# zhaowenlan1779/hekaton-system

Measured on AMD Instinct MI355X. Metric: subcircuit Groth16 proofs/sec (whole node), big-merkle, higher is better.
Workload: dtype u32 limbs (Montgomery mod-p integers)

## Files before the change

hekaton_system_amd/csrc/ntt.cuh:

```cuda
#pragma once
#include "field.cuh"

namespace hk {

constexpr int NTT_TILE_LOG = 11;
constexpr int NTT_THREADS = 512;
constexpr int POW_TABLE_BITS = 11;
constexpr int POW_TABLE_SIZE = 1 << POW_TABLE_BITS;

#if defined(__HIPCC__)

template <class Fr>
__device__ __forceinline__ Fr fr_load(const Fr* p) {
    Fr r;
    const uint4* s = reinterpret_cast<const uint4*>(p);
    uint4 a = s[0], b = s[1];
    r.v[0] = a.x; r.v[1] = a.y; r.v[2] = a.z; r.v[3] = a.w;
    r.v[4] = b.x; r.v[5] = b.y; r.v[6] = b.z; r.v[7] = b.w;
    return r;
}
template <class Fr>
__device__ __forceinline__ void fr_store(Fr* p, const Fr& lazy) {
    Fr r = Fr::canon(lazy);
    uint4* d = reinterpret_cast<uint4*>(p);
// ... 9 lines not shown
    for (u32 k = 0; k < nbits; k++)
        if ((i >> k) & 1) acc = Fr::mul(acc, fr_load(&sq[k]));
    fr_store(&tw[i], acc);
}

template <class Fr>
__device__ __forceinline__ Fr pow_from_tables(const Fr* __restrict__ pw, u32 j, u32 logn) {
    Fr g = fr_load(&pw[j & (POW_TABLE_SIZE - 1)]);
    if (logn > POW_TABLE_BITS) g = Fr::mul(g, fr_load(&pw[POW_TABLE_SIZE + ((j >> POW_TABLE_BITS) & (POW_TABLE_SIZE - 1))]));
    if (logn > 2 * POW_TABLE_BITS) g = Fr::mul(g, fr_load(&pw[2 * POW_TABLE_SIZE + (j >> (2 * POW_TABLE_BITS))]));
    return g;
}

template <class Fr>
__global__ void k_stage_tables(Fr* __restrict__ tws, const Fr* __restrict__ tw, u32 log_table) {
    size_t i = (size_t)blockIdx.x * blockDim.x + threadIdx.x;
    if ((i + 1) >> log_table) return;
    u32 s = 31 - __clz((u32)(i + 1));
    size_t j = i + 1 - ((size_t)1 << s);
    fr_store(&tws[i], fr_load(&tw[j << (log_table - s - 1)]));
}

template <class Fr, int DIT>
__global__ void __launch_bounds__(NTT_THREADS)
k_ntt_pass4(Fr* __restrict__ data, size_t stride_vec, const Fr* __restrict__ tws, u32 logn, u32 lo, u32 nst,
            u32 cols_bits, int post, u32 npost, Fr scale, const Fr* __restrict__ pw, const Fr* __restrict__ sub,
            Fr kc) {
    extern __shared__ uint4 lds_raw[];
    Fr* lds = reinterpret_cast<Fr*>(lds_raw);
    const u32 nthr = blockDim.x;
    if (blockIdx.y >= npost) post = 0;
    Fr* vec = data + (size_t)blockIdx.y * stride_vec;
    const u32 cols = 1u << cols_bits;
    const u32 tile_elems = 1u << (nst + cols_bits);
    const u32 mid_bits = lo - cols_bits;
    const u32 mid = blockIdx.x & ((1u << mid_bits) - 1u);
    const size_t base = ((size_t)(blockIdx.x >> mid_bits) << (lo + nst)) | ((size_t)mid << cols_bits);
    for (u32 e = threadIdx.x; e < tile_elems; e += nthr) {
        u32 r = e >> cols_bits, c = e & (cols - 1);
        lds[e] = fr_load(&vec[base | ((size_t)r << lo) | c]);
    }
    __syncthreads();
    const u32 npair = nst >> 1;
    for (u32 k = 0; k < npair; k++) {
        const u32 l = DIT ? 2 * k : nst - 2 - 2 * k;
        const u32 s = lo + l;
        const Fr* t_lo = tws + (((size_t)1 << s) - 1);
        const Fr* t_hi = tws + (((size_t)2 << s) - 1);
        for (u32 q = threadIdx.x; q < (tile_elems >> 2); q += nthr) {
            u32 c = q & (cols - 1), rr = q >> cols_bits;
            u32 r0 = ((rr >> l) << (l + 2)) | (rr & ((1u << l) - 1u));
            u32 j = (u32)((base | ((size_t)r0 << lo) | c) & (((size_t)1 << s) - 1));
            Fr wc = fr_load(&t_lo[j]);
            Fr wa = fr_load(&t_hi[j]);
            Fr wb = fr_load(&t_hi[j + (1u << s)]);
            u32 i0 = (r0 << cols_bits) | c, st = 1u << (l + cols_bits);
            Fr x0 = lds[i0], x1 = lds[i0 + st], x2 = lds[i0 + 2 * st], x3 = lds[i0 + 3 * st];
            if (DIT) {
                Fr v = Fr::mul(x1, wc), u = Fr::mul(x3, wc);
                x1 = Fr::sub(x0, v); x0 = Fr::add(x0, v);
                x3 = Fr::sub(x2, u); x2 = Fr::add(x2, u);
                v = Fr::mul(x2, wa); u = Fr::mul(x3, wb);
                x2 = Fr::sub(x0, v); x0 = Fr::add(x0, v);
                x3 = Fr::sub(x1, u); x1 = Fr::add(x1, u);
            } else {
                Fr v = Fr::sub(x0, x2), u = Fr::sub(x1, x3);
                x0 = Fr::add(x0, x2); x1 = Fr::add(x1, x3);
                x2 = Fr::mul(v, wa); x3 = Fr::mul(u, wb);
                v = Fr::sub(x0, x1); u = Fr::sub(x2, x3);
                x0 = Fr::add(x0, x1); x2 = Fr::add(x2, x3);
                x1 = Fr::mul(v, wc); x3 = Fr::mul(u, wc);
            }
            lds[i0] = x0; lds[i0 + st] = x1; lds[i0 + 2 * st] = x2; lds[i0 + 3 * st] = x3;
        }
        __syncthreads();
    }
    if (nst & 1) {
        const u32 l = DIT ? nst - 1 : 0;
        const u32 s = lo + l;
        const Fr* t_lo = tws + (((size_t)1 << s) - 1);
        for (u32 q = threadIdx.x; q < (tile_elems >> 1); q += nthr) {
            u32 c = q & (cols - 1), rr = q >> cols_bits;
            u32 r0 = ((rr >> l) << (l + 1)) | (rr & ((1u << l) - 1u));
            u32 j = (u32)((base | ((size_t)r0 << lo) | c) & (((size_t)1 << s) - 1));
            Fr w = fr_load(&t_lo[j]);
            u32 i0 = (r0 << cols_bits) | c, st = 1u << (l + cols_bits);
            Fr x0 = lds[i0], x1 = lds[i0 + st];
            if (DIT) {
                Fr v = Fr::mul(x1, w);
                lds[i0] = Fr::add(x0, v);
                lds[i0 + st] = Fr::sub(x0, v);
            } else {
                lds[i0] = Fr::add(x0, x1);
                lds[i0 + st] = Fr::mul(Fr::sub(x0, x1), w);
            }
        }
        __syncthreads();
    }
    for (u32 e = threadIdx.x; e < tile_elems; e += nthr) {
        u32 r = e >> cols_bits, c = e & (cols - 1);
        size_t gi = base | ((size_t)r << lo) | c;
        Fr x = lds[e];
        if (post & 2) x = Fr::mul(x, pow_from_tables(pw, logn ? (__brev((u32)gi) >> (32 - logn)) : 0u, logn));
        if (post & 4) x = Fr::sub(x, Fr::mul(fr_load(&sub[gi]), kc));
        if (post & 1) x = Fr::mul(x, scale);
        fr_store(&vec[gi], x);
    }
}

template <class Fr>
__global__ void k_scale_pow(Fr* __restrict__ data, size_t stride_vec, const Fr* __restrict__ pw, Fr scale,
                            u32 logn, int bitrev_index, int use_pow) {
    size_t pos = (size_t)blockIdx.x * blockDim.x + threadIdx.x;
    if (pos >> logn) return;
    Fr* vec = data + (size_t)blockIdx.y * stride_vec;
    Fr x = fr_load(&vec[pos]);
    x = Fr::mul(x, scale);
    if (use_pow) {
        u32 j = bitrev_index ? (logn ? (__brev((u32)pos) >> (32 - logn)) : 0u) : (u32)pos;
        x = Fr::mul(x, pow_from_tables(pw, j, logn));
    }
    fr_store(&vec[pos], x);
}

template <class Fr>
__global__ void k_bitrev(Fr* __restrict__ data, u32 logn) {
    size_t pos = (size_t)blockIdx.x * blockDim.x + threadIdx.x;
    if (pos >> logn) return;
    u32 r = logn ? (__brev((u32)pos) >> (32 - logn)) : 0u;
// ... 6 lines not shown

template <class Fr>
__global__ void k_spmv(const u64* __restrict__ row_ptr, const u32* __restrict__ col,
                       const Fr* __restrict__ val, const Fr* __restrict__ z, Fr* __restrict__ out,
                       u32 n_rows, u32 n_copy, u32 m) {
    u32 row = blockIdx.x * blockDim.x + threadIdx.x;
    if (row >= m) return;
    if (row >= n_rows) {
        fr_store(&out[row], row - n_rows < n_copy ? fr_load(&z[row - n_rows]) : Fr::zero());
        return;
    }
    u64 b = row_ptr[row], e = row_ptr[row + 1];
    Fr acc = Fr::zero();
    Fr one = Fr::one();
    for (u64 k = b; k < e; k++) {
        Fr c = fr_load(&val[k]);
        Fr x = fr_load(&z[col[k]]);
        if (!(c == one)) x = Fr::mul(x, c);
        acc = Fr::add(acc, x);
    }
    fr_store(&out[row], acc);
}

template <int UNUSED>
__global__ void k_csr_check(const u64* __restrict__ row_ptr, const u32* __restrict__ col, u64 n_rows, u64 nnz,
                            u32 n_cols, u32* __restrict__ bad) {
    u64 t = (u64)blockIdx.x * blockDim.x + threadIdx.x, stride = (u64)gridDim.x * blockDim.x;
    u32 f = 0;
    for (u64 i = t; i < n_rows; i += stride) {
        u64 b = row_ptr[i], e = row_ptr[i + 1];
        if (b > e || e > nnz) f = 1;
    }
    for (u64 k = t; k < nnz; k += stride)
        if (col[k] >= n_cols) f = 2;
    if (t == 0 && (row_ptr[0] != 0 || row_ptr[n_rows] != nnz)) f = 3;
    if (f) atomicOr(bad, f);
}

template <class Fr>
__global__ void k_copy_inputs(Fr* __restrict__ a, const Fr* __restrict__ z, u32 n_c, u32 n_inst) {
    u32 j = blockIdx.x * blockDim.x + threadIdx.x;
    if (j < n_inst) fr_store(&a[n_c + j], fr_load(&z[j]));
}

template <class Fr>
__global__ void k_mul_pointwise(Fr* __restrict__ a, const Fr* __restrict__ b, size_t m) {
// ... 9 lines not shown
```

hekaton_system_amd/csrc/prove_impl.cuh:

```cuda
#pragma once
#include <string>
#include "curve_ops_impl.cuh"
#include "ntt.cuh"
#include "fixed_base.cuh"
#include "witness.cuh"
#include "endo.cuh"

namespace hk {

template <class Fr>
static Fr host_halve(const Fr& a) {
    u32 t[Fr::N + 1];
    u64 c = 0;
    bool odd = a.v[0] & 1;
    for (int i = 0; i < Fr::N; i++) {
        c += (u64)a.v[i] + (odd ? Fr::Params::MOD[i] : 0u);
        t[i] = (u32)c;
        c >>= 32;
    }
    t[Fr::N] = (u32)c;
    Fr r;
    for (int i = 0; i < Fr::N; i++) r.v[i] = (t[i] >> 1) | (t[i + 1] << 31);
    return r;
}
template <class Fr>
static Fr host_from_limbs(const u32* l) {
    Fr r;
    for (int i = 0; i < Fr::N; i++) r.v[i] = l[i];
    return r;
}

struct NttTables {
    std::mutex mu;
    u32 log_table = 0;
    void* tw_fwd = nullptr;
    void* tw_inv = nullptr;
    void* pw_g = nullptr;
    void* pw_ginv = nullptr;
    std::vector<void*> retired;
};

template <class C>
struct NttHost {
    typedef typename C::Fr Fr;

    static hk_status ensure(hk_ctx* ctx, u32 log_m, NttTables** out) {
        if (log_m > C::TWO_ADICITY) return HK_ERR_DOMAIN_TOO_LARGE;
        std::unique_lock<std::mutex> lk(ctx->mu);
        if (!ctx->ntt) ctx->ntt = new NttTables();
        NttTables* T = ctx->ntt;
        lk.unlock();
        std::unique_lock<std::mutex> tl(T->mu);
        *out = T;
        if (T->log_table >= log_m && T->tw_fwd) return HK_OK;
        u32 L = log_m < 16 ? 16 : log_m;
        if (L > C::TWO_ADICITY) L = C::TWO_ADICITY;
        HK_HIP(hipSetDevice(ctx->device));
        std::vector<Fr> sq(32), sqi(32);
        Fr w = host_from_limbs<Fr>(C::ROOT);
        for (u32 k = 0; k < C::TWO_ADICITY - L; k++) w = Fr::sqr(w);
        Fr winv = Fr::one();
// ... 42 lines not shown
        return HK_OK;
    }

    static Fr size_inv(u32 log_m) {
        Fr x = Fr::one();
        for (u32 k = 0; k < log_m; k++) x = host_halve(x);
        return x;
    }
    static Fr vanishing_inv_on_coset(u32 log_m) {
        Fr g = host_from_limbs<Fr>(C::GEN);
        for (u32 k = 0; k < log_m; k++) g = Fr::sqr(g);
        return fp_inv(Fr::sub(g, Fr::one()));
    }

    struct Post {
        int post = 0;
        u32 nvec = 0xffffffffu;
        const Fr* scale = nullptr;
        const Fr* pw = nullptr;
        const Fr* sub = nullptr;
        const Fr* kc = nullptr;
    };

    static hk_status passes(hipStream_t s, Fr* data, size_t stride, u32 batch, u32 logn, const Fr* tws, int dit,
                            const Post& ep = Post()) {
        if (logn == 0) return HK_OK;
        static const u32 upper_max = [] {
            const char* e = getenv("HK_NTT_UPPER_MAX");
            u32 v = e ? (u32)atoi(e) : 6u;
            return v < 1 ? 1u : (v > 10 ? 10u : v);
        }();
        static const u32 tile_log = [] {
            const char* e = getenv("HK_NTT_TILE_LOG");
            u32 v = e ? (u32)atoi(e) : (u32)NTT_TILE_LOG;
            return v < 8 ? 8u : (v > (u32)NTT_TILE_LOG ? (u32)NTT_TILE_LOG : v);
        }();
        const u32 threads = 1u << (tile_log - 2);
        u32 bottom = logn < tile_log ? logn : tile_log;
        u32 rest = logn - bottom;
        u32 npass = (rest + upper_max - 1) / upper_max;
        struct P { u32 lo, nst, cols_bits; } ps[34];
        int np = 0;
        ps[np++] = {0, bottom, 0};
        u32 lo = bottom;
        for (u32 i = 0; i < npass; i++) {
            u32 nst = (rest - (lo - bottom) + (npass - i) - 1) / (npass - i);
            ps[np++] = {lo, nst, tile_log - nst};
            lo += nst;
        }
        Fr one = Fr::one();
        for (int k = 0; k < np; k++) {
            const P& p = dit ? ps[k] : ps[np - 1 - k];
            u32 tile_log = p.nst + p.cols_bits;
            dim3 grid(1u << (logn - tile_log), batch);
            size_t lds = sizeof(Fr) << tile_log;
            bool last = k == np - 1;
            int pp = last ? ep.post : 0;
            const Fr& sc = (pp & 1) ? *ep.scale : one;
            const Fr& kc = (pp & 4) ? *ep.kc : one;
            if (dit)
                hipLaunchKernelGGL((k_ntt_pass4<Fr, 1>), grid, dim3(threads), lds, s, data, stride, tws, logn, p.lo,
                                   p.nst, p.cols_bits, pp, ep.nvec, sc, ep.pw, ep.sub, kc);
            else
                hipLaunchKernelGGL((k_ntt_pass4<Fr, 0>), grid, dim3(threads), lds, s, data, stride, tws, logn, p.lo,
                                   p.nst, p.cols_bits, pp, ep.nvec, sc, ep.pw, ep.sub, kc);
        }
        HK_HIP(hipGetLastError());
        return HK_OK;
    }

    static hk_status scale(hipStream_t s, Fr* data, size_t stride, u32 batch, u32 logn, const Fr* pw,
                           const Fr& sc, int bitrev_index, int use_pow) {
        size_t n = (size_t)1 << logn;
        hipLaunchKernelGGL((k_scale_pow<Fr>), dim3((u32)((n + 255) / 256), batch), dim3(256), 0, s, data,
                           stride, pw, sc, logn, bitrev_index, use_pow);
        HK_HIP(hipGetLastError());
        return HK_OK;
    }
    static hk_status bitrev(hipStream_t s, Fr* data, u32 logn) {
        size_t n = (size_t)1 << logn;
        hipLaunchKernelGGL((k_bitrev<Fr>), dim3((u32)((n + 255) / 256)), dim3(256), 0, s, data, logn);
        HK_HIP(hipGetLastError());
        return HK_OK;
    }
};

template <class C>
hk_status Ops<C>::ntt(hk_ctx* ctx, void* data, unsigned log_m, int inverse, int coset) {
    typedef NttHost<C> N;
    NttTables* T;
// ... 35 lines not shown
    HK_HIP(hipMemsetAsync(flag, 0, sizeof(u32), s));
    size_t work = M.n_rows > M.nnz ? M.n_rows : M.nnz;
    u32 blocks = (u32)std::min<size_t>((work + 255) / 256, 2048);
    if (blocks == 0) blocks = 1;
    hipLaunchKernelGGL((k_csr_check<0>), dim3(blocks), dim3(256), 0, s, M.row_ptr, M.col, (u64)M.n_rows, (u64)M.nnz,
                       (u32)n_cols, flag);
    u32 h = 0;
    HK_HIP(hipMemcpyAsync(&h, flag, sizeof(u32), hipMemcpyDeviceToHost, s));
    HK_HIP(hipStreamSynchronize(s));
    return h ? HK_ERR_ARG : HK_OK;
}

template <class C>
struct QapHost {
    typedef typename C::Fr Fr;
    typedef NttHost<C> N;

    static u32 domain_log(size_t n_c, size_t n_inst) {
        size_t need = n_c + n_inst;
        u32 lg = 0;
        while (((size_t)1 << lg) < need) lg++;
        return lg;
    }
    static hk_status run(hipStream_t s, NttTables* T, const CsrDev& A, const CsrDev& B, const CsrDev& Cm,
                         size_t n_inst, size_t n_c, const Fr* z, Fr* abc, u32 log_m) {
        size_t m = (size_t)1 << log_m;
        const CsrDev* Ms[3] = {&A, &B, &Cm};
        for (int k = 0; k < 3; k++) {
            hipLaunchKernelGGL((k_spmv<Fr>), dim3((u32)((m + 255) / 256)), dim3(256), 0, s,
                               Ms[k]->row_ptr, Ms[k]->col, (const Fr*)Ms[k]->val, z, abc + k * m,
                               (u32)n_c, k == 0 ? (u32)n_inst : 0u, (u32)m);
        }
        const Fr* tinv = (const Fr*)T->tw_inv;
        const Fr* tfwd = (const Fr*)T->tw_fwd;
        typename N::Post e1;
        e1.post = 2;
        e1.nvec = 2;
        e1.pw = (const Fr*)T->pw_g;
        HK_TRY(N::passes(s, abc, m, 3, log_m, tinv, 0, e1));
        HK_TRY(N::passes(s, abc, m, 2, log_m, tfwd, 1));
        hipLaunchKernelGGL((k_mul_pointwise<Fr>), dim3((u32)((m + 255) / 256)), dim3(256), 0, s, abc, abc + m, m);
        Fr minv = N::size_inv(log_m);
        Fr mm = fp_inv(Fr::mul(minv, minv));
        Fr k = Fr::mul(N::vanishing_inv_on_coset(log_m), Fr::mul(minv, Fr::mul(minv, minv)));
        typename N::Post e2;
        e2.post = 2 | 4 | 1;
        e2.pw = (const Fr*)T->pw_ginv;
        e2.sub = abc + 2 * m;
        e2.kc = &mm;
        e2.scale = &k;
        HK_TRY(N::passes(s, abc, m, 1, log_m, tinv, 0, e2));
        HK_HIP(hipGetLastError());
        return HK_OK;
    }
};

template <class C>
hk_status Ops<C>::witness_map(hk_ctx* ctx, const hk_csr* A, const hk_csr* B, const hk_csr* Cm, size_t n_inst,
                              size_t n_c, const void* z, size_t n_v, void* h_out, size_t h_cap,
                              size_t* m_out) {
    typedef QapHost<C> Q;
    if (A->n_rows != n_c || B->n_rows != n_c || Cm->n_rows != n_c || n_inst > n_v || n_inst < 1) return HK_ERR_ARG;
    for (auto M : {A, B, Cm})
        if (!M->row_ptr || (M->nnz && (!M->col || !M->val_mont))) return HK_ERR_ARG;
    u32 log_m = Q::domain_log(n_c, n_inst);
    if (log_m > C::TWO_ADICITY) return HK_ERR_DOMAIN_TOO_LARGE;
    size_t m = (size_t)1 << log_m;
    if (m_out) *m_out = m;
    if (h_cap < m) return HK_ERR_LEN;
    NttTables* T;
    HK_TRY(NttHost<C>::ensure(ctx, log_m, &T));
    LaneGuard g(ctx);
    Lane* L = g.lane;
    if (!L) return HK_ERR_DEVICE;
    const hk_csr* Ms[3] = {A, B, Cm};
    const void *rp[3], *cl[3], *vl[3], *zd;
    u32* flag;
    Fr* abc;
    HK_TRY(L->carve([&](Carve& c) {
        for (int k = 0; k < 3; k++) {
            rp[k] = c.take(8 * (Ms[k]->n_rows + 1));
            cl[k] = c.take(4 * Ms[k]->nnz);
            vl[k] = c.take(sizeof(Fr) * Ms[k]->nnz);
        }
        flag = c.n<u32>(1);
        zd = c.take(n_v * sizeof(Fr));
        abc = c.n<Fr>(3 * m);
    }));
    CsrDev D[3];
    for (int k = 0; k < 3; k++) {
        HK_TRY(to_device(L, Ms[k]->row_ptr, 8 * (Ms[k]->n_rows + 1), &rp[k]));
        HK_TRY(to_device(L, Ms[k]->col, 4 * Ms[k]->nnz, &cl[k]));
        HK_TRY(to_device(L, Ms[k]->val_mont, sizeof(Fr) * Ms[k]->nnz, &vl[k]));
        D[k] = {(const u64*)rp[k], (const u32*)cl[k], vl[k], Ms[k]->n_rows, Ms[k]->nnz};
// ... 965 lines not shown
                HK_HIP(hipMemcpyAsync(t, src, k * sizeof(F), hipMemcpyHostToDevice, L->stream));
                sd = t;
            }
            F* dd = out_dev ? dst : u;
            hipLaunchKernelGGL(k_field_convert<F>, dim3((unsigned)((k + 255) / 256)), dim3(256), 0, L->stream, sd, dd, k, to_mont);
            HK_HIP(hipGetLastError());
            if (!out_dev) HK_HIP(hipMemcpyAsync(dst, dd, k * sizeof(F), hipMemcpyDeviceToHost, L->stream));
            HK_TRY(L->settle());
        }
        return HK_OK;
    };
    return which == 0 ? run(Fr()) : run(Fq());
}

template <class C>
void Ops<C>::ctx_release(hk_ctx* ctx) {
    for (auto& e : ctx->fb_cache)
        if (e.table) (void)hipFree(e.table);
    ctx->fb_cache.clear();
    if (!ctx->ntt) return;
    NttTables* T = ctx->ntt;
    for (void* p : {T->tw_fwd, T->tw_inv, T->pw_g, T->pw_ginv})
        if (p) (void)hipFree(p);
    for (void* p : T->retired) (void)hipFree(p);
    delete T;
    ctx->ntt = nullptr;
}

template <class Fr>
__global__ void k_prep_ext(Fr* __restrict__ ext, u32 ext_stride, const Fr* __restrict__ rs_kappas, u32 rs_stride,
                           u32 n_kappas, u32 batch, u32* __restrict__ c0, u32* __restrict__ c1, u32* __restrict__ c2,
                           u32 nb0, u32 nb1, u32 nb2) {
    u32 gt = blockIdx.x * blockDim.x + threadIdx.x, stride = gridDim.x * blockDim.x;
    for (u32 i = gt; i < nb0; i += stride) c0[i] = 0;
    for (u32 i = gt; i < nb1; i += stride) c1[i] = 0;
    for (u32 i = gt; i < nb2; i += stride) c2[i] = 0;
    if (gt >= batch) return;
    Fr* e = ext + (size_t)gt * ext_stride;
    const Fr* rk = rs_kappas + (size_t)gt * rs_stride;
    Fr r = fr_load(&rk[0]), s = fr_load(&rk[1]);
    fr_store(&e[0], r);
    fr_store(&e[1], s);
    fr_store(&e[2], Fr::mul(r, s));
    for (u32 i = 0; i < n_kappas; i++) fr_store(&e[3 + i], fr_load(&rk[2 + i]));
}

// ... 180 lines not shown
    }
    return HK_OK;
}

template <class C>
hk_status Ops<C>::prove_batch(hk_ctx* ctx, const hk_pk* h, size_t n_v, size_t n_kappas, const ProveRow* rows, size_t batch) {
    typedef QapHost<C> Q;
    if (h->ctx != ctx) return HK_ERR_ARG;
    PkImpl<C>* pk = (PkImpl<C>*)h->impl;
    if (!pk->has_qap) return HK_ERR_ARG;
    if (n_v != pk->n_v) return HK_ERR_LEN;
    if (n_kappas + 1 != pk->n_stages) return HK_ERR_LEN;
    if (batch == 0) return HK_OK;
    if (!rows) return HK_ERR_ARG;
    for (size_t b = 0; b < batch; b++) {
        const ProveRow& w = rows[b];
        if (!w.z || !w.r || !w.s || !w.a || !w.b || !w.c || (n_kappas && !w.kappas)) return HK_ERR_ARG;
    }
    LaneGuard g(ctx, ProveLaneTag{});
    Lane* L = g.lane;
    if (!L) return HK_ERR_DEVICE;
    NttTables* T;
    HK_TRY(NttHost<C>::ensure(ctx, pk->log_m, &T));
    const MsmPlan &pz = pk->plan_z, &ph = pk->plan_h, &pb = pk->plan_b;
    const size_t m = (size_t)1 << pk->log_m, fr = sizeof(Fr), rs_stride = 2 + n_kappas;
    std::vector<char> z_dev(batch);
    bool any_host = false;
    for (size_t b = 0; b < batch; b++) {
        z_dev[b] = is_device_ptr(rows[b].z);
        any_host = any_host || !z_dev[b];
    }
    Fr *zext, *small, *zt, *zb, *abc;
    SortBufs sb, sbh, sbb;
    typename MsmRun<Fq>::Bufs rbA, rbB1, rbL, rbh;
    typename MsmRun<Fq2>::Bufs rb2;
    XYZZ<Fq>* res1;
    XYZZ<Fq2>* res2;
    Affine<Fq> *oa, *oc;
    Affine<Fq2>* ob;
    XYZZ<Fq>* pc;
    auto chunk_bufs = [&](Carve& c, u32 nb) {
        zext = c.n<Fr>((size_t)pk->n_ext * nb);
        small = c.n<Fr>(rs_stride * nb);
        zt = any_host ? c.n<Fr>(n_v * nb) : nullptr;
        MsmSort<Fr>::alloc(c, pz, &sb, nb);
        MsmSort<Fr>::alloc(c, ph, &sbh, nb);
// ... 19 lines not shown
    size_t chunk = batch < (size_t)HK_PROVE_BATCH_CHUNK ? batch : (size_t)HK_PROVE_BATCH_CHUNK;
    if (chunk > 1) {
        size_t free_b = 0, total_b = 0;
        if (hipMemGetInfo(&free_b, &total_b) != hipSuccess) { (void)hipGetLastError(); free_b = 0; }
        size_t avail = free_b + L->arena_cap;
        auto chunk_bytes = [&](size_t nb) { Carve c; chunk_bufs(c, (u32)nb); return c.off; };
        while (chunk > 1 && chunk_bytes(chunk) > avail) chunk--;
    }
    std::vector<unsigned char> rsk(batch * rs_stride * fr);
    for (size_t b = 0; b < batch; b++) {
        unsigned char* row = rsk.data() + b * rs_stride * fr;
        memcpy(row, rows[b].r, fr);
        memcpy(row + fr, rows[b].s, fr);
        if (n_kappas) memcpy(row + 2 * fr, rows[b].kappas, n_kappas * fr);
    }
    std::vector<Affine<Fq>> ha(chunk), hc(chunk);
    std::vector<Affine<Fq2>> hb(chunk);
    std::vector<const Fr*> zd(chunk);
    const bool prof = ctx->profiling;
    hipEvent_t* ev = L->ev;
    hk_timings acc;
    memset(&acc, 0, sizeof(acc));
    static const EndoSplit<2> endo_g1 = EndoOf<Fq>::split();
    hipStream_t rs[PROVE_ROLES];
    for (int r = 0; r < PROVE_ROLES; r++) rs[r] = L->stream_at(prove_role_stream(L->n_streams, (ProveRole)r));
    hipStream_t s = rs[ROLE_MAIN];
    auto wait = [](hipStream_t to, hipEvent_t e, hipStream_t from) -> hk_status {
        if (to != from) HK_HIP(hipStreamWaitEvent(to, e, 0));
        return HK_OK;
    };
    for (size_t b0 = 0; b0 < batch; b0 += chunk) {
        const u32 nb = (u32)std::min(chunk, batch - b0);
        HK_TRY(L->carve([&](Carve& c) { chunk_bufs(c, nb); }));
        hipEvent_t ev_start = b0 ? ev[9] : ev[0];
        if (prof) HK_HIP(hipEventRecord(ev_start, s));
        for (u32 j = 0; j < nb; j++) {
            if (z_dev[b0 + j]) zd[j] = (const Fr*)rows[b0 + j].z;
            else {
                HK_HIP(hipMemcpyAsync(zt + (size_t)j * n_v, rows[b0 + j].z, n_v * fr, hipMemcpyHostToDevice, s));
                zd[j] = zt + (size_t)j * n_v;
            }
            if (n_v > 1)
                HK_HIP(hipMemcpyAsync(zext + (size_t)j * pk->n_ext, zd[j] + 1, (n_v - 1) * fr, hipMemcpyDeviceToDevice, s));
        }
        HK_HIP(hipMemcpyAsync(small, rsk.data() + b0 * rs_stride * fr, nb * rs_stride * fr, hipMemcpyHostToDevice, s));
        hipLaunchKernelGGL((k_prep_ext<Fr>), dim3(64), dim3(256), 0, s, zext + (n_v - 1), pk->n_ext, (const Fr*)small,
                           (u32)rs_stride, (u32)n_kappas, nb, sb.count, sbh.count, sbb.count, pz.NB * nb, ph.NB * nb,
                           pk->b_compact ? pb.NB * nb : 0u);
        hipStream_t sB1 = rs[ROLE_B1], sB2 = rs[ROLE_B2], sL = rs[ROLE_L], sH = rs[ROLE_H];
        hipEvent_t ev_z = ev[16], ev_sorted = ev[17];
        HK_HIP(hipEventRecord(ev_z, s));
        auto submit_h = [&]() -> hk_status {
            HK_TRY(wait(sH, ev_z, s));
            if (prof) HK_HIP(hipEventRecord(ev[5], sH));
            for (u32 j = 0; j < nb; j++)
                HK_TRY(Q::run(sH, T, pk->csr[0], pk->csr[1], pk->csr[2], pk->n_inst, pk->n_c, zd[j],
                              abc + (size_t)j * 3 * m, pk->log_m));
            if (prof) HK_HIP(hipEventRecord(ev[6], sH));
            HK_TRY(MsmSort<Fr>::run(sH, ph, (const u32*)abc, 1, sbh, true, nb, 3 * m));
            HK_TRY(MsmRun<Fq>::run(sH, ph, pk->h_tab, (u32)m, 0, sbh, rbh, res1 + 3, prof ? ev[12] : nullptr,
                                   prof ? ev[13] : nullptr, nb, 4));
            HK_HIP(hipEventRecord(ev[7], sH));
            return HK_OK;
        };
        const bool h_first = L->n_streams >= 3;
        if (h_first) HK_TRY(submit_h());
        HK_TRY(MsmSort<Fr>::run(s, pz, (const u32*)zext, 1, sb, true, nb, pk->n_ext));
        HK_HIP(hipEventRecord(ev_sorted, s));
        if (prof) HK_HIP(hipEventRecord(ev[1], s));
        HK_TRY(wait(sL, ev_sorted, s));
        const SortBufs* sbB = &sb;
        if (pk->b_compact) {
            HK_TRY(wait(sB1, ev_z, s));
            hipLaunchKernelGGL((k_gather<Fr>), dim3((pk->b_n + 255) / 256, nb), dim3(256), 0, sB1, zb, (const Fr*)zext,
                               (const u32*)pk->b_idx, pk->b_n, pk->n_ext);
            HK_TRY(MsmSort<Fr>::run(sB1, pb, (const u32*)zb, 1, sbb, true, nb, pk->b_n));
            HK_HIP(hipEventRecord(ev[28], sB1));
            HK_TRY(wait(sB2, ev[28], sB1));
            sbB = &sbb;
        } else {
            HK_TRY(wait(sB1, ev_sorted, s));
// ... 12 lines not shown
        if (prof) HK_HIP(hipEventRecord(ev[2], s));
        HK_TRY(wait(s, ev[3], sB1));
        HK_TRY(wait(s, ev[4], sB2));
        HK_TRY(wait(s, ev[18], sL));
        hipLaunchKernelGGL((k_finish_ab<Fr, Fq, Fq2>), dim3(3, nb), dim3(64), 0, s, res1, res2, pk->consts_g1, pk->consts_g2,
                           (const Fr*)small, (u32)rs_stride, oa, ob, pc, endo_g1);
        HK_HIP(hipGetLastError());
        if (!h_first) HK_TRY(submit_h());
        HK_TRY(wait(s, ev[7], sH));
        if (prof) HK_HIP(hipEventRecord(ev[19], s));
        hipLaunchKernelGGL((k_finish_c<Fq>), dim3(1), dim3(64), 0, s, (const XYZZ<Fq>*)pc, (const XYZZ<Fq>*)res1, oc, nb);
        HK_HIP(hipGetLastError());
        HK_HIP(hipMemcpyAsync(ha.data(), oa, nb * sizeof(Affine<Fq>), hipMemcpyDeviceToHost, s));
        HK_HIP(hipMemcpyAsync(hb.data(), ob, nb * sizeof(Affine<Fq2>), hipMemcpyDeviceToHost, s));
        HK_HIP(hipMemcpyAsync(hc.data(), oc, nb * sizeof(Affine<Fq>), hipMemcpyDeviceToHost, s));
        if (prof) HK_HIP(hipEventRecord(ev[8], s));
        HK_TRY(L->settle());
        for (u32 j = 0; j < nb; j++) {
            memcpy(rows[b0 + j].a, &ha[j], sizeof(Affine<Fq>));
            memcpy(rows[b0 + j].b, &hb[j], sizeof(Affine<Fq2>));
            memcpy(rows[b0 + j].c, &hc[j], sizeof(Affine<Fq>));
        }
        if (prof) {
            acc.digits_ms += ev_ms(ev_start, ev[1]);
            acc.msm_a_ms += ev_ms(ev[1], ev[2]);
            hipEvent_t fork_b = pk->b_compact ? ev_z : ev[1];
            acc.msm_b_g1_ms += ev_ms(fork_b, ev[3]);
            acc.msm_b_g2_ms += ev_ms(fork_b, ev[4]);
            acc.msm_l_ms += ev_ms(ev[1], ev[18]);
            acc.witness_map_ms += ev_ms(ev[5], ev[6]);
            acc.msm_h_ms += ev_ms(ev[6], ev[7]);
            acc.finish_ms += ev_ms(ev[19], ev[8]);
            float kh = ev_ms(ev[12], ev[13]);
            acc.accum_h_ms += kh;
            acc.accum_kernel_ms += kh + ev_ms(ev[22], ev[23]) + ev_ms(ev[24], ev[25]) + ev_ms(ev[26], ev[27]);
            acc.accum_kernel_launches += 4;
        }
    }
    if (prof) {
        acc.total_ms = ev_ms(ev[0], ev[8]);
        acc.batch_proofs = (uint32_t)chunk;
        L->timings = acc;
    }
    return HK_OK;
}

}
// ... 3 lines not shown
```

Baseline: 125.0.

## Fuse witness-map NTT seams, batch SpMV, and skip trivial twiddle multiplies

Restructures the witness-map (H polynomial) pipeline. Adjacent inverse and forward NTT passes at the bottom and top seams are fused into single kernels, so one kernel does inverse NTT, coset shift and forward NTT on an LDS-resident tile. The top seam also folds the pointwise A*B product and the following inverse NTT into one kernel. The three SpMVs become one launch, the closing scale is folded into a precomputed power table, and stage-0 butterflies skip multiplies by one. This removes several global-memory round trips and kernel launches, at the cost of more complex kernels and a new plan helper. It also adds an optional split of the witness maps onto the main stream.

```diff
diff --git a/hekaton_system_amd/csrc/ntt.cuh b/hekaton_system_amd/csrc/ntt.cuh
--- a/hekaton_system_amd/csrc/ntt.cuh
+++ b/hekaton_system_amd/csrc/ntt.cuh
@@ -55,31 +55,42 @@
 }
 
 template <class Fr, int DIT>
-__global__ void __launch_bounds__(NTT_THREADS)
-k_ntt_pass4(Fr* __restrict__ data, size_t stride_vec, const Fr* __restrict__ tws, u32 logn, u32 lo, u32 nst,
-            u32 cols_bits, int post, u32 npost, Fr scale, const Fr* __restrict__ pw, const Fr* __restrict__ sub,
-            Fr kc) {
-    extern __shared__ uint4 lds_raw[];
-    Fr* lds = reinterpret_cast<Fr*>(lds_raw);
-    const u32 nthr = blockDim.x;
-    if (blockIdx.y >= npost) post = 0;
-    Fr* vec = data + (size_t)blockIdx.y * stride_vec;
+__device__ __forceinline__ void ntt_tile_stages(Fr* lds, const Fr* __restrict__ tws, size_t base, u32 lo, u32 nst,
+                                                u32 cols_bits, u32 nthr) {
     const u32 cols = 1u << cols_bits;
     const u32 tile_elems = 1u << (nst + cols_bits);
-    const u32 mid_bits = lo - cols_bits;
-    const u32 mid = blockIdx.x & ((1u << mid_bits) - 1u);
-    const size_t base = ((size_t)(blockIdx.x >> mid_bits) << (lo + nst)) | ((size_t)mid << cols_bits);
-    for (u32 e = threadIdx.x; e < tile_elems; e += nthr) {
-        u32 r = e >> cols_bits, c = e & (cols - 1);
-        lds[e] = fr_load(&vec[base | ((size_t)r << lo) | c]);
-    }
-    __syncthreads();
     const u32 npair = nst >> 1;
     for (u32 k = 0; k < npair; k++) {
         const u32 l = DIT ? 2 * k : nst - 2 - 2 * k;
         const u32 s = lo + l;
         const Fr* t_lo = tws + (((size_t)1 << s) - 1);
         const Fr* t_hi = tws + (((size_t)2 << s) - 1);
+        if (s == 0) {
+            const Fr w4 = fr_load(&t_hi[1]);
+            for (u32 q = threadIdx.x; q < (tile_elems >> 2); q += nthr) {
+                u32 c = q & (cols - 1), rr = q >> cols_bits;
+                u32 i0 = (rr << (2 + cols_bits)) | c, st = cols;
+                Fr x0 = lds[i0], x1 = lds[i0 + st], x2 = lds[i0 + 2 * st], x3 = lds[i0 + 3 * st];
+                if (DIT) {
+                    Fr v = x1, u = x3;
+                    x1 = Fr::sub(x0, v); x0 = Fr::add(x0, v);
+                    x3 = Fr::sub(x2, u); x2 = Fr::add(x2, u);
+                    v = x2; u = Fr::mul(x3, w4);
+                    x2 = Fr::sub(x0, v); x0 = Fr::add(x0, v);
+                    x3 = Fr::sub(x1, u); x1 = Fr::add(x1, u);
+                } else {
+                    Fr v = Fr::sub(x0, x2), u = Fr::sub(x1, x3);
+                    x0 = Fr::add(x0, x2); x1 = Fr::add(x1, x3);
+                    x2 = v; x3 = Fr::mul(u, w4);
+                    v = Fr::sub(x0, x1); u = Fr::sub(x2, x3);
+                    x0 = Fr::add(x0, x1); x2 = Fr::add(x2, x3);
+                    x1 = v; x3 = u;
+                }
+                lds[i0] = x0; lds[i0 + st] = x1; lds[i0 + 2 * st] = x2; lds[i0 + 3 * st] = x3;
+            }
+            __syncthreads();
+            continue;
+        }
         for (u32 q = threadIdx.x; q < (tile_elems >> 2); q += nthr) {
             u32 c = q & (cols - 1), rr = q >> cols_bits;
             u32 r0 = ((rr >> l) << (l + 2)) | (rr & ((1u << l) - 1u));
@@ -115,10 +126,15 @@
         for (u32 q = threadIdx.x; q < (tile_elems >> 1); q += nthr) {
             u32 c = q & (cols - 1), rr = q >> cols_bits;
             u32 r0 = ((rr >> l) << (l + 1)) | (rr & ((1u << l) - 1u));
+            u32 i0 = (r0 << cols_bits) | c, st = 1u << (l + cols_bits);
+            Fr x0 = lds[i0], x1 = lds[i0 + st];
+            if (s == 0) {
+                lds[i0] = Fr::add(x0, x1);
+                lds[i0 + st] = Fr::sub(x0, x1);
+                continue;
+            }
             u32 j = (u32)((base | ((size_t)r0 << lo) | c) & (((size_t)1 << s) - 1));
             Fr w = fr_load(&t_lo[j]);
-            u32 i0 = (r0 << cols_bits) | c, st = 1u << (l + cols_bits);
-            Fr x0 = lds[i0], x1 = lds[i0 + st];
             if (DIT) {
                 Fr v = Fr::mul(x1, w);
                 lds[i0] = Fr::add(x0, v);
@@ -130,6 +146,29 @@
         }
         __syncthreads();
     }
+}
+
+template <class Fr, int DIT>
+__global__ void __launch_bounds__(NTT_THREADS)
+k_ntt_pass4(Fr* __restrict__ data, size_t stride_vec, const Fr* __restrict__ tws, u32 logn, u32 lo, u32 nst,
+            u32 cols_bits, int post, u32 npost, Fr scale, const Fr* __restrict__ pw, const Fr* __restrict__ sub,
+            Fr kc) {
+    extern __shared__ uint4 lds_raw[];
+    Fr* lds = reinterpret_cast<Fr*>(lds_raw);
+    const u32 nthr = blockDim.x;
+    if (blockIdx.y >= npost) post = 0;
+    Fr* vec = data + (size_t)blockIdx.y * stride_vec;
+    const u32 cols = 1u << cols_bits;
+    const u32 tile_elems = 1u << (nst + cols_bits);
+    const u32 mid_bits = lo - cols_bits;
+    const u32 mid = blockIdx.x & ((1u << mid_bits) - 1u);
+    const size_t base = ((size_t)(blockIdx.x >> mid_bits) << (lo + nst)) | ((size_t)mid << cols_bits);
+    for (u32 e = threadIdx.x; e < tile_elems; e += nthr) {
+        u32 r = e >> cols_bits, c = e & (cols - 1);
+        lds[e] = fr_load(&vec[base | ((size_t)r << lo) | c]);
+    }
+    __syncthreads();
+    ntt_tile_stages<Fr, DIT>(lds, tws, base, lo, nst, cols_bits, nthr);
     for (u32 e = threadIdx.x; e < tile_elems; e += nthr) {
         u32 r = e >> cols_bits, c = e & (cols - 1);
         size_t gi = base | ((size_t)r << lo) | c;
@@ -138,6 +177,66 @@
         if (post & 4) x = Fr::sub(x, Fr::mul(fr_load(&sub[gi]), kc));
         if (post & 1) x = Fr::mul(x, scale);
         fr_store(&vec[gi], x);
+    }
+}
+
+template <class Fr>
+__global__ void __launch_bounds__(NTT_THREADS)
+k_ntt_seam_bottom(Fr* __restrict__ data, size_t stride_vec, const Fr* __restrict__ tinv, const Fr* __restrict__ tfwd,
+                  u32 logn, u32 nst, u32 ndit, const Fr* __restrict__ pw) {
+    extern __shared__ uint4 lds_raw[];
+    Fr* lds = reinterpret_cast<Fr*>(lds_raw);
+    const u32 nthr = blockDim.x;
+    Fr* vec = data + (size_t)blockIdx.y * stride_vec;
+    const u32 tile_elems = 1u << nst;
+    const size_t base = (size_t)blockIdx.x << nst;
+    for (u32 e = threadIdx.x; e < tile_elems; e += nthr) lds[e] = fr_load(&vec[base + e]);
+    __syncthreads();
+    ntt_tile_stages<Fr, 0>(lds, tinv, base, 0, nst, 0, nthr);
+    if (blockIdx.y < ndit) {
+        for (u32 e = threadIdx.x; e < tile_elems; e += nthr)
+            lds[e] = Fr::mul(lds[e], pow_from_tables(pw, __brev((u32)(base + e)) >> (32 - logn), logn));
+        __syncthreads();
+        ntt_tile_stages<Fr, 1>(lds, tfwd, base, 0, nst, 0, nthr);
+    }
+    for (u32 e = threadIdx.x; e < tile_elems; e += nthr) fr_store(&vec[base + e], lds[e]);
+}
+
+template <class Fr>
+__global__ void __launch_bounds__(NTT_THREADS)
+k_ntt_seam_top(Fr* __restrict__ a, const Fr* __restrict__ b, const Fr* __restrict__ tfwd,
+               const Fr* __restrict__ tinv, u32 lo, u32 nst, u32 cols_bits) {
+    extern __shared__ uint4 lds_raw[];
+    Fr* lds = reinterpret_cast<Fr*>(lds_raw);
+    const u32 nthr = blockDim.x;
+    const u32 cols = 1u << cols_bits;
+    const u32 mid_bits = lo - cols_bits;
+    const u32 mid = blockIdx.x & ((1u << mid_bits) - 1u);
+    const size_t base = ((size_t)(blockIdx.x >> mid_bits) << (lo + nst)) | ((size_t)mid << cols_bits);
+    Fr ra[4];
+    HK_UNROLL for (u32 k = 0; k < 4; k++) {
+        u32 e = threadIdx.x + k * nthr, r = e >> cols_bits, c = e & (cols - 1);
+        lds[e] = fr_load(&a[base | ((size_t)r << lo) | c]);
+    }
+    __syncthreads();
+    ntt_tile_stages<Fr, 1>(lds, tfwd, base, lo, nst, cols_bits, nthr);
+    HK_UNROLL for (u32 k = 0; k < 4; k++) ra[k] = lds[threadIdx.x + k * nthr];
+    __syncthreads();
+    HK_UNROLL for (u32 k = 0; k < 4; k++) {
+        u32 e = threadIdx.x + k * nthr, r = e >> cols_bits, c = e & (cols - 1);
+        lds[e] = fr_load(&b[base | ((size_t)r << lo) | c]);
+    }
+    __syncthreads();
+    ntt_tile_stages<Fr, 1>(lds, tfwd, base, lo, nst, cols_bits, nthr);
+    HK_UNROLL for (u32 k = 0; k < 4; k++) {
+        u32 e = threadIdx.x + k * nthr;
+        lds[e] = Fr::mul(ra[k], lds[e]);
+    }
+    __syncthreads();
+    ntt_tile_stages<Fr, 0>(lds, tinv, base, lo, nst, cols_bits, nthr);
+    HK_UNROLL for (u32 k = 0; k < 4; k++) {
+        u32 e = threadIdx.x + k * nthr, r = e >> cols_bits, c = e & (cols - 1);
+        fr_store(&a[base | ((size_t)r << lo) | c], lds[e]);
     }
 }
 
@@ -190,6 +289,32 @@
     fr_store(&out[row], acc);
 }
 
+struct SpmvMats { const u64* row_ptr[3]; const u32* col[3]; const void* val[3]; };
+template <class Fr>
+__global__ void k_spmv3(SpmvMats M, const Fr* __restrict__ z, Fr* __restrict__ out, u32 n_rows, u32 n_copy, u32 m) {
+    u32 row = blockIdx.x * blockDim.x + threadIdx.x;
+    if (row >= m) return;
+    const u32 y = blockIdx.y;
+    out += (size_t)y * m;
+    if (row >= n_rows) {
+        fr_store(&out[row], (y == 0 && row - n_rows < n_copy) ? fr_load(&z[row - n_rows]) : Fr::zero());
+        return;
+    }
+    const u64* row_ptr = y == 0 ? M.row_ptr[0] : y == 1 ? M.row_ptr[1] : M.row_ptr[2];
+    const u32* col = y == 0 ? M.col[0] : y == 1 ? M.col[1] : M.col[2];
+    const Fr* val = (const Fr*)(y == 0 ? M.val[0] : y == 1 ? M.val[1] : M.val[2]);
+    u64 b = row_ptr[row], e = row_ptr[row + 1];
+    Fr acc = Fr::zero();
+    Fr one = Fr::one();
+    for (u64 k = b; k < e; k++) {
+        Fr c = fr_load(&val[k]);
+        Fr x = fr_load(&z[col[k]]);
+        if (!(c == one)) x = Fr::mul(x, c);
+        acc = Fr::add(acc, x);
+    }
+    fr_store(&out[row], acc);
+}
+
 template <int UNUSED>
 __global__ void k_csr_check(const u64* __restrict__ row_ptr, const u32* __restrict__ col, u64 n_rows, u64 nnz,
                             u32 n_cols, u32* __restrict__ bad) {
diff --git a/hekaton_system_amd/csrc/prove_impl.cuh b/hekaton_system_amd/csrc/prove_impl.cuh
--- a/hekaton_system_amd/csrc/prove_impl.cuh
+++ b/hekaton_system_amd/csrc/prove_impl.cuh
@@ -2,6 +2,7 @@
 #include <string>
 #include "curve_ops_impl.cuh"
 #include "ntt.cuh"
+#include "wm_plan.h"
 #include "fixed_base.cuh"
 #include "witness.cuh"
 #include "endo.cuh"
@@ -37,6 +38,7 @@
     void* tw_inv = nullptr;
     void* pw_g = nullptr;
     void* pw_ginv = nullptr;
+    void* pw_close[33] = {};
     std::vector<void*> retired;
 };
 
@@ -125,50 +127,62 @@
         const Fr* kc = nullptr;
     };
 
-    static hk_status passes(hipStream_t s, Fr* data, size_t stride, u32 batch, u32 logn, const Fr* tws, int dit,
-                            const Post& ep = Post()) {
-        if (logn == 0) return HK_OK;
-        static const u32 upper_max = [] {
+    static u32 upper_max() {
+        static const u32 v = [] {
             const char* e = getenv("HK_NTT_UPPER_MAX");
             u32 v = e ? (u32)atoi(e) : 6u;
             return v < 1 ? 1u : (v > 10 ? 10u : v);
         }();
-        static const u32 tile_log = [] {
+        return v;
+    }
+    static u32 tile_log() {
+        static const u32 v = [] {
             const char* e = getenv("HK_NTT_TILE_LOG");
             u32 v = e ? (u32)atoi(e) : (u32)NTT_TILE_LOG;
             return v < 8 ? 8u : (v > (u32)NTT_TILE_LOG ? (u32)NTT_TILE_LOG : v);
         }();
-        const u32 threads = 1u << (tile_log - 2);
-        u32 bottom = logn < tile_log ? logn : tile_log;
-        u32 rest = logn - bottom;
-        u32 npass = (rest + upper_max - 1) / upper_max;
-        struct P { u32 lo, nst, cols_bits; } ps[34];
-        int np = 0;
-        ps[np++] = {0, bottom, 0};
-        u32 lo = bottom;
-        for (u32 i = 0; i < npass; i++) {
-            u32 nst = (rest - (lo - bottom) + (npass - i) - 1) / (npass - i);
-            ps[np++] = {lo, nst, tile_log - nst};
-            lo += nst;
-        }
+        return v;
+    }
+
+    static void pass(hipStream_t s, Fr* data, size_t stride, u32 batch, u32 logn, const Fr* tws, int dit, const NttPass& p,
+                     int pp, const Post& ep) {
+        const u32 threads = 1u << (tile_log() - 2);
+        u32 tl = p.nst + p.cols_bits;
+        dim3 grid(1u << (logn - tl), batch);
+        size_t lds = sizeof(Fr) << tl;
         Fr one = Fr::one();
-        for (int k = 0; k < np; k++) {
-            const P& p = dit ? ps[k] : ps[np - 1 - k];
-            u32 tile_log = p.nst + p.cols_bits;
-            dim3 grid(1u << (logn - tile_log), batch);
-            size_t lds = sizeof(Fr) << tile_log;
-            bool last = k == np - 1;
-            int pp = last ? ep.post : 0;
-            const Fr& sc = (pp & 1) ? *ep.scale : one;
-            const Fr& kc = (pp & 4) ? *ep.kc : one;
-            if (dit)
-                hipLaunchKernelGGL((k_ntt_pass4<Fr, 1>), grid, dim3(threads), lds, s, data, stride, tws, logn, p.lo,
-                                   p.nst, p.cols_bits, pp, ep.nvec, sc, ep.pw, ep.sub, kc);
-            else
-                hipLaunchKernelGGL((k_ntt_pass4<Fr, 0>), grid, dim3(threads), lds, s, data, stride, tws, logn, p.lo,
-                                   p.nst, p.cols_bits, pp, ep.nvec, sc, ep.pw, ep.sub, kc);
-        }
+        const Fr& sc = (pp & 1) ? *ep.scale : one;
+        const Fr& kc = (pp & 4) ? *ep.kc : one;
+        if (dit)
+            hipLaunchKernelGGL((k_ntt_pass4<Fr, 1>), grid, dim3(threads), lds, s, data, stride, tws, logn, p.lo,
+                               p.nst, p.cols_bits, pp, ep.nvec, sc, ep.pw, ep.sub, kc);
+        else
+            hipLaunchKernelGGL((k_ntt_pass4<Fr, 0>), grid, dim3(threads), lds, s, data, stride, tws, logn, p.lo,
+                               p.nst, p.cols_bits, pp, ep.nvec, sc, ep.pw, ep.sub, kc);
+    }
+
+    static hk_status passes(hipStream_t s, Fr* data, size_t stride, u32 batch, u32 logn, const Fr* tws, int dit,
+                            const Post& ep = Post()) {
+        if (logn == 0) return HK_OK;
+        const NttPassPlan pl = ntt_pass_plan(logn, tile_log(), upper_max());
+        for (int k = 0; k < pl.np; k++)
+            pass(s, data, stride, batch, logn, tws, dit, dit ? pl.ps[k] : pl.ps[pl.np - 1 - k], k == pl.np - 1 ? ep.post : 0, ep);
         HK_HIP(hipGetLastError());
+        return HK_OK;
+    }
+
+    static hk_status ensure_close(hk_ctx* ctx, NttTables* T, u32 log_m, const Fr& k) {
+        std::unique_lock<std::mutex> tl(T->mu);
+        if (log_m > 32 || T->pw_close[log_m]) return HK_OK;
+        HK_HIP(hipSetDevice(ctx->device));
+        Fr* pc = nullptr;
+        HK_HIP(hipMalloc((void**)&pc, sizeof(Fr) * 3 * POW_TABLE_SIZE));
+        HK_HIP(hipMemcpy(pc, T->pw_ginv, sizeof(Fr) * 3 * POW_TABLE_SIZE, hipMemcpyDeviceToDevice));
+        hipLaunchKernelGGL((k_scale_pow<Fr>), dim3(POW_TABLE_SIZE / 256, 1), dim3(256), 0, 0, pc, (size_t)0, (const Fr*)nullptr,
+                           k, (u32)POW_TABLE_BITS, 0, 0);
+        HK_HIP(hipGetLastError());
+        HK_HIP(hipDeviceSynchronize());
+        T->pw_close[log_m] = pc;
         return HK_OK;
     }
 
@@ -250,15 +264,74 @@
         while (((size_t)1 << lg) < need) lg++;
         return lg;
     }
+    static bool fused() {
+        static const bool v = [] {
+            const char* e = getenv("HK_WM_FUSE");
+            return !(e && atoi(e) == 0) && N::tile_log() == (u32)NTT_TILE_LOG && N::upper_max() == 6u;
+        }();
+        return v;
+    }
+    static Fr closing_scale(u32 log_m) {
+        Fr minv = N::size_inv(log_m);
+        return Fr::mul(N::vanishing_inv_on_coset(log_m), Fr::mul(minv, Fr::mul(minv, minv)));
+    }
+    static hk_status prepare(hk_ctx* ctx, NttTables* T, u32 log_m) {
+        if (!fused()) return HK_OK;
+        return N::ensure_close(ctx, T, log_m, closing_scale(log_m));
+    }
     static hk_status run(hipStream_t s, NttTables* T, const CsrDev& A, const CsrDev& B, const CsrDev& Cm,
                          size_t n_inst, size_t n_c, const Fr* z, Fr* abc, u32 log_m) {
+        if (!fused()) return run_unfused(s, T, A, B, Cm, n_inst, n_c, z, abc, log_m);
+        if (log_m > 32 || !T->pw_close[log_m]) return HK_ERR_DEVICE;
+        size_t m = (size_t)1 << log_m;
+        SpmvMats M = {{A.row_ptr, B.row_ptr, Cm.row_ptr}, {A.col, B.col, Cm.col}, {A.val, B.val, Cm.val}};
+        hipLaunchKernelGGL((k_spmv3<Fr>), dim3((u32)((m + 255) / 256), 3), dim3(256), 0, s, M, z, abc, (u32)n_c, (u32)n_inst,
+                           (u32)m);
+        const Fr* tinv = (const Fr*)T->tw_inv;
+        const Fr* tfwd = (const Fr*)T->tw_fwd;
+        Fr minv = N::size_inv(log_m);
+        Fr mmk = Fr::mul(fp_inv(Fr::mul(minv, minv)), closing_scale(log_m));
+        typename N::Post e0, e2;
+        e2.post = 2 | 4;
+        e2.pw = (const Fr*)T->pw_close[log_m];
+        e2.sub = abc + 2 * m;
+        e2.kc = &mmk;
+        const WmPlan w = wm_plan(log_m, N::tile_log(), N::upper_max(), true);
+        const u32 threads = 1u << (N::tile_log() - 2);
+        for (int i = 0; i < w.n; i++) {
+            const WmStep& st = w.steps[i];
+            const NttPass& p = w.passes.ps[st.pass];
+            const u32 tl = p.nst + p.cols_bits;
+            switch (st.kind) {
+            case WM_PASS:
+                if (st.transform == 0) N::pass(s, abc, m, 3, log_m, tinv, 0, p, 0, e0);
+                else if (st.transform == 1) N::pass(s, abc, m, 2, log_m, tfwd, 1, p, 0, e0);
+                else N::pass(s, abc, m, 1, log_m, tinv, 0, p, st.last ? e2.post : 0, e2);
+                break;
+            case WM_SEAM_BOTTOM:
+                hipLaunchKernelGGL((k_ntt_seam_bottom<Fr>), dim3(1u << (log_m - tl), 3), dim3(threads), sizeof(Fr) << tl, s, abc,
+                                   m, tinv, tfwd, log_m, p.nst, 2u, (const Fr*)T->pw_g);
+                break;
+            case WM_SEAM_TOP:
+                hipLaunchKernelGGL((k_ntt_seam_top<Fr>), dim3(1u << (log_m - tl)), dim3(threads), sizeof(Fr) << tl, s, abc,
+                                   (const Fr*)(abc + m), tfwd, tinv, p.lo, p.nst, p.cols_bits);
+                break;
+            case WM_MUL:
+                hipLaunchKernelGGL((k_mul_pointwise<Fr>), dim3((u32)((m + 255) / 256)), dim3(256), 0, s, abc, abc + m, m);
+                break;
+            }
+        }
+        HK_HIP(hipGetLastError());
+        return HK_OK;
+    }
+    static hk_status run_unfused(hipStream_t s, NttTables* T, const CsrDev& A, const CsrDev& B, const CsrDev& Cm,
+                                 size_t n_inst, size_t n_c, const Fr* z, Fr* abc, u32 log_m) {
         size_t m = (size_t)1 << log_m;
         const CsrDev* Ms[3] = {&A, &B, &Cm};
-        for (int k = 0; k < 3; k++) {
+        for (int k = 0; k < 3; k++)
             hipLaunchKernelGGL((k_spmv<Fr>), dim3((u32)((m + 255) / 256)), dim3(256), 0, s,
                                Ms[k]->row_ptr, Ms[k]->col, (const Fr*)Ms[k]->val, z, abc + k * m,
                                (u32)n_c, k == 0 ? (u32)n_inst : 0u, (u32)m);
-        }
         const Fr* tinv = (const Fr*)T->tw_inv;
         const Fr* tfwd = (const Fr*)T->tw_fwd;
         typename N::Post e1;
@@ -270,7 +343,7 @@
         hipLaunchKernelGGL((k_mul_pointwise<Fr>), dim3((u32)((m + 255) / 256)), dim3(256), 0, s, abc, abc + m, m);
         Fr minv = N::size_inv(log_m);
         Fr mm = fp_inv(Fr::mul(minv, minv));
-        Fr k = Fr::mul(N::vanishing_inv_on_coset(log_m), Fr::mul(minv, Fr::mul(minv, minv)));
+        Fr k = closing_scale(log_m);
         typename N::Post e2;
         e2.post = 2 | 4 | 1;
         e2.pw = (const Fr*)T->pw_ginv;
@@ -298,6 +371,7 @@
     if (h_cap < m) return HK_ERR_LEN;
     NttTables* T;
     HK_TRY(NttHost<C>::ensure(ctx, log_m, &T));
+    HK_TRY(Q::prepare(ctx, T, log_m));
     LaneGuard g(ctx);
     Lane* L = g.lane;
     if (!L) return HK_ERR_DEVICE;
@@ -1309,6 +1383,8 @@
     NttTables* T = ctx->ntt;
     for (void* p : {T->tw_fwd, T->tw_inv, T->pw_g, T->pw_ginv})
         if (p) (void)hipFree(p);
+    for (void* p : T->pw_close)
+        if (p) (void)hipFree(p);
     for (void* p : T->retired) (void)hipFree(p);
     delete T;
     ctx->ntt = nullptr;
@@ -1535,6 +1611,7 @@
     if (!L) return HK_ERR_DEVICE;
     NttTables* T;
     HK_TRY(NttHost<C>::ensure(ctx, pk->log_m, &T));
+    HK_TRY(Q::prepare(ctx, T, pk->log_m));
     const MsmPlan &pz = pk->plan_z, &ph = pk->plan_h, &pb = pk->plan_b;
     const size_t m = (size_t)1 << pk->log_m, fr = sizeof(Fr), rs_stride = 2 + n_kappas;
     std::vector<char> z_dev(batch);
@@ -1600,6 +1677,10 @@
     hk_timings acc;
     memset(&acc, 0, sizeof(acc));
     static const EndoSplit<2> endo_g1 = EndoOf<Fq>::split();
+    static const u32 wm_split = [] {
+        const char* e = getenv("HK_PROVE_WM_SPLIT");
+        return e ? (u32)std::max(0, atoi(e)) : 0u;
+    }();
     hipStream_t rs[PROVE_ROLES];
     for (int r = 0; r < PROVE_ROLES; r++) rs[r] = L->stream_at(prove_role_stream(L->n_streams, (ProveRole)r));
     hipStream_t s = rs[ROLE_MAIN];
@@ -1628,13 +1709,26 @@
         hipStream_t sB1 = rs[ROLE_B1], sB2 = rs[ROLE_B2], sL = rs[ROLE_L], sH = rs[ROLE_H];
         hipEvent_t ev_z = ev[16], ev_sorted = ev[17];
         HK_HIP(hipEventRecord(ev_z, s));
+        const u32 k_main = std::min(nb, wm_split);
+        auto run_maps = [&](hipStream_t st, u32 j0, u32 j1) -> hk_status {
+            for (u32 j = j0; j < j1; j++)
+                HK_TRY(Q::run(st, T, pk->csr[0], pk->csr[1], pk->csr[2], pk->n_inst, pk->n_c, zd[j],
+                              abc + (size_t)j * 3 * m, pk->log_m));
+            return HK_OK;
+        };
+        hipEvent_t ev_digits = ev_start;
+        if (k_main) {
+            if (prof) HK_HIP(hipEventRecord(ev[14], s));
+            HK_TRY(run_maps(s, nb - k_main, nb));
+            HK_HIP(hipEventRecord(ev[10], s));
+            if (prof) ev_digits = ev[10];
+        }
         auto submit_h = [&]() -> hk_status {
             HK_TRY(wait(sH, ev_z, s));
             if (prof) HK_HIP(hipEventRecord(ev[5], sH));
-            for (u32 j = 0; j < nb; j++)
-                HK_TRY(Q::run(sH, T, pk->csr[0], pk->csr[1], pk->csr[2], pk->n_inst, pk->n_c, zd[j],
-                              abc + (size_t)j * 3 * m, pk->log_m));
+            HK_TRY(run_maps(sH, 0, nb - k_main));
             if (prof) HK_HIP(hipEventRecord(ev[6], sH));
+            if (k_main) HK_TRY(wait(sH, ev[10], s));
             HK_TRY(MsmSort<Fr>::run(sH, ph, (const u32*)abc, 1, sbh, true, nb, 3 * m));
             HK_TRY(MsmRun<Fq>::run(sH, ph, pk->h_tab, (u32)m, 0, sbh, rbh, res1 + 3, prof ? ev[12] : nullptr,
                                    prof ? ev[13] : nullptr, nb, 4));
@@ -1693,7 +1787,7 @@
             memcpy(rows[b0 + j].c, &hc[j], sizeof(Affine<Fq>));
         }
         if (prof) {
-            acc.digits_ms += ev_ms(ev_start, ev[1]);
+            acc.digits_ms += ev_ms(ev_digits, ev[1]) + (k_main ? ev_ms(ev_start, ev[14]) : 0.f);
             acc.msm_a_ms += ev_ms(ev[1], ev[2]);
             hipEvent_t fork_b = pk->b_compact ? ev_z : ev[1];
             acc.msm_b_g1_ms += ev_ms(fork_b, ev[3]);
diff --git a/hekaton_system_amd/csrc/wm_plan.h b/hekaton_system_amd/csrc/wm_plan.h
--- /dev/null
+++ b/hekaton_system_amd/csrc/wm_plan.h
@@ -0,0 +1,65 @@
+#pragma once
+
+namespace hk {
+
+struct NttPass { unsigned lo, nst, cols_bits; };
+enum { NTT_MAX_PASSES = 34 };
+struct NttPassPlan {
+    int np = 0;
+    NttPass ps[NTT_MAX_PASSES] = {};
+};
+
+inline NttPassPlan ntt_pass_plan(unsigned logn, unsigned tile_log, unsigned upper_max) {
+    NttPassPlan pl;
+    if (logn == 0) return pl;
+    unsigned bottom = logn < tile_log ? logn : tile_log;
+    unsigned rest = logn - bottom;
+    unsigned npass = (rest + upper_max - 1) / upper_max;
+    pl.ps[pl.np++] = {0, bottom, 0};
+    unsigned lo = bottom;
+    for (unsigned i = 0; i < npass; i++) {
+        unsigned nst = (rest - (lo - bottom) + (npass - i) - 1) / (npass - i);
+        pl.ps[pl.np++] = {lo, nst, tile_log - nst};
+        lo += nst;
+    }
+    return pl;
+}
+
+enum WmStepKind { WM_PASS = 0, WM_SEAM_BOTTOM, WM_SEAM_TOP, WM_MUL };
+struct WmStep {
+    WmStepKind kind;
+    int transform;
+    int pass;
+    bool last;
+};
+struct WmPlan {
+    NttPassPlan passes;
+    bool fuse_bottom = false, fuse_top = false;
+    int n = 0;
+    WmStep steps[3 * NTT_MAX_PASSES + 1];
+};
+
+inline WmPlan wm_plan(unsigned logn, unsigned tile_log, unsigned upper_max, bool fuse) {
+    WmPlan w;
+    w.passes = ntt_pass_plan(logn, tile_log, upper_max);
+    const int np = w.passes.np;
+    w.fuse_bottom = fuse && np >= 1;
+    w.fuse_top = fuse && np >= 2;
+    for (int k = np - 1; k >= 0; k--) {
+        if (k == 0 && w.fuse_bottom) w.steps[w.n++] = {WM_SEAM_BOTTOM, 0, 0, false};
+        else w.steps[w.n++] = {WM_PASS, 0, k, k == 0};
+    }
+    for (int k = 0; k < np; k++) {
+        if (k == 0 && w.fuse_bottom) continue;
+        if (k == np - 1 && w.fuse_top) w.steps[w.n++] = {WM_SEAM_TOP, 1, k, false};
+        else w.steps[w.n++] = {WM_PASS, 1, k, k == np - 1};
+    }
+    if (!w.fuse_top) w.steps[w.n++] = {WM_MUL, 1, 0, false};
+    for (int k = np - 1; k >= 0; k--) {
+        if (k == np - 1 && w.fuse_top) continue;
+        w.steps[w.n++] = {WM_PASS, 2, k, k == 0};
+    }
+    return w;
+}
+
+}
```

Result: faster. 126.8 (median of 6 runs) (+1.4%).
